# sieste/greb-climate-model

Hardware: AMD Instinct MI355X
Metric: simulated-years/sec at 96x48 grid (ensemble aggregate); diffusion HBM GB/s vs roofline (higher is better)
Workload: dtype f32; 1 GPU; 96x48 GREB ensemble, 512 members/GPU x 1 GPU, CO2 sweep 280-1120 ppm, 33 scenario years after 1 flux-correction year, dt=12h, dt_crcl=0.5h; members_per_gpu=512, arithmetic=fast, gather=none (1 GPU)

## Files before the change

### greb_climate_model_amd/csrc/greb_device.h

```cpp
#pragma once
#include <hip/hip_runtime.h>

namespace greb {

constexpr int kMaxNy = 192;

struct RowTables {
  float dif_ccy, adv_ccy;
  float dif_ccx[kMaxNy], adv_ccx[kMaxNy];
  float dif_ccx2[kMaxNy], adv_ccx2[kMaxNy];
  int dif_time2[kMaxNy], adv_time2[kMaxNy];
  int subcycled[kMaxNy];
};

struct f4 {
  float v[4];
};

typedef __attribute__((address_space(3))) float lfloat;
typedef float vfloat4 __attribute__((ext_vector_type(4)));

__device__ __forceinline__ f4 ld4(const float* p) {
  const vfloat4 a = *reinterpret_cast<const vfloat4*>(p);
  return f4{{a.x, a.y, a.z, a.w}};
}
__device__ __forceinline__ f4 ld4(const lfloat* p) {
  const vfloat4 a = *(const __attribute__((address_space(3))) vfloat4*)p;
  return f4{{a.x, a.y, a.z, a.w}};
}
__device__ __forceinline__ void st4(float* p, const f4& a) {
  vfloat4 v; v.x = a.v[0]; v.y = a.v[1]; v.z = a.v[2]; v.w = a.v[3];
  *reinterpret_cast<vfloat4*>(p) = v;
}
__device__ __forceinline__ f4 ld4_nt(const float* p) {
  const vfloat4 a = __builtin_nontemporal_load(reinterpret_cast<const vfloat4*>(p));
  return f4{{a.x, a.y, a.z, a.w}};
}
__device__ __forceinline__ void st4_nt(float* p, const f4& a) {
  vfloat4 v; v.x = a.v[0]; v.y = a.v[1]; v.z = a.v[2]; v.w = a.v[3];
  __builtin_nontemporal_store(v, reinterpret_cast<vfloat4*>(p));
}
__device__ __forceinline__ void st4(lfloat* p, const f4& a) {
  vfloat4 v; v.x = a.v[0]; v.y = a.v[1]; v.z = a.v[2]; v.w = a.v[3];
  *(__attribute__((address_space(3))) vfloat4*)p = v;
}

__device__ __forceinline__ f4 zero4() { return f4{{0.f, 0.f, 0.f, 0.f}}; }

template <typename P>
__device__ __forceinline__ void load_window(P row, int q, int nq, float t[12]) {
  const int qm = (q == 0) ? nq - 1 : q - 1;
  const int qp = (q == nq - 1) ? 0 : q + 1;
  const f4 a = ld4(row + 4 * qm), b = ld4(row + 4 * q), c = ld4(row + 4 * qp);
#pragma unroll
  for (int i = 0; i < 4; ++i) { t[i] = a.v[i]; t[4 + i] = b.v[i]; t[8 + i] = c.v[i]; }
}

__device__ __forceinline__ float min3f(float a, float b, float c) {
  float r;
  asm("v_min3_f32 %0, %1, %2, %3" : "=v"(r) : "v"(a), "v"(b), "v"(c));
  return r;
}

__device__ __forceinline__ float split_m(float u) { return u >= 0.0f ? u : 0.0f; }
__device__ __forceinline__ float split_p(float u) { return u >= 0.0f ? 0.0f : u; }


typedef float v2 __attribute__((ext_vector_type(2)));
__device__ __forceinline__ float fma_e(float a, float b, float c) { return __builtin_fmaf(a, b, c); }
__device__ __forceinline__ v2 fma_e(v2 a, v2 b, v2 c) { return __builtin_elementwise_fma(a, b, c); }
__device__ __forceinline__ float splat_e(float x, float) { return x; }
__device__ __forceinline__ v2 splat_e(float x, v2) { return v2{x, x}; }
__device__ __forceinline__ float clamp_e(float d, float T) {
#pragma clang fp contract(off)
  return (d <= -T) ? -0.9f * T : d;
}
__device__ __forceinline__ v2 clamp_e(v2 d, v2 T) { return v2{clamp_e(d.x, T.x), clamp_e(d.y, T.y)}; }

template <typename E>
__device__ __forceinline__ E div_by_const(E x, float c, float r) {
#pragma clang fp contract(off)
  const E q = x * r;
  const E e = fma_e(-q, splat_e(c, x), x);
  return fma_e(e, splat_e(r, x), q);
}
template <typename E> __device__ __forceinline__ E div20(E x) { return div_by_const(x, 20.f, 1.0f / 20.f); }
template <typename E> __device__ __forceinline__ E div3(E x) { return div_by_const(x, 3.f, 1.0f / 3.f); }

template <typename E>
__device__ __forceinline__ E dif_S_strict(const E* T, const E* w, int c) {
#pragma clang fp contract(off)
  return 10.f * (w[c - 1] * (T[c - 1] - T[c]) + w[c + 1] * (T[c + 1] - T[c]))
         + 4.f * (w[c - 2] * (T[c - 2] - T[c - 1]) + w[c - 1] * (T[c] - T[c - 1]))
         + 4.f * (w[c + 1] * (T[c] - T[c + 1]) + w[c + 2] * (T[c + 2] - T[c + 1]))
         + (w[c - 3] * (T[c - 3] - T[c - 2]) + w[c - 2] * (T[c - 1] - T[c - 2]))
         + (w[c + 2] * (T[c + 1] - T[c + 2]) + w[c + 3] * (T[c + 3] - T[c + 2]));
}

template <typename E>
__device__ __forceinline__ void dif_lon_strict(const E T[12], const E w[12], float cc, E d[4]) {
// ... 310 lines not shown
```

### greb_climate_model_amd/csrc/greb_member.hip

```cpp
#include <cstdlib>

#include "greb_kernels.h"
#include "greb_pair.h"
#include "greb_physics_step.h"
#include "greb_stencil.h"

namespace greb {

constexpr int NX = 96, NY = 48, NQ = 24, NP = 4608;
constexpr int kThreads = 512;
constexpr int RS = 2 * NX + 16;
constexpr int XB = (NY + 2) * RS;
constexpr int kOffX = RS;
constexpr int kOffW = 2 * XB + RS;
constexpr int kOffWX = 3 * XB;
constexpr int kOffWY = kOffWX + NP;
constexpr int kOffRowK = kOffWY + NP;
constexpr int kLdsFloats = kOffRowK + NY * kRowKWords;
constexpr size_t kLdsBytes = (size_t)kLdsFloats * sizeof(float);

bool member_layout_supported(const RowTables& t, int nx, int ny) {
  if (nx != NX || ny != NY) return false;
  for (int k = 0; k < NY; ++k) {
    const bool sub = (k <= 9 || k >= 38);
// ... 218 lines not shown
              "a deal must cover 3 ST, 3 FT, 1 S1 and 5 F1 passes exactly once");

__host__ __device__ constexpr int pass_tasks(int kind, int index) {
  const int total = kind == kST || kind == kFT ? 8 * NQ : (kind == kS1 ? 2 * NQ : (kind == kF1 ? 12 * NQ : 0));
  const int left = total - 64 * index;
  return left >= 64 ? 64 : (left > 0 ? left : 0);
}

template <bool STRICT>
__device__ __forceinline__ BulkTasks make_tasks(int wave, int lane) {
  BulkTasks b;
#pragma unroll
  for (int i = 0; i < 3; ++i) {
    int k = 1, q = 0, valid = 0;
    {
      const int kind = deal<STRICT>(wave, i).kind, t = deal<STRICT>(wave, i).index * 64 + lane;
      const int r = t / NQ;
      q = t % NQ;
      if (kind == kST) { valid = r < 8; k = r < 4 ? 1 + 2 * r : (r == 4 ? 41 : (r == 5 ? 39 : (r == 6 ? 45 : 43))); }
      else if (kind == kFT) { valid = r < 8; k = 10 + 2 * r; }
      else if (kind == kS1) { valid = r < 2; k = r == 0 ? 9 : 38; if (r == 1) q = (q + 4) % NQ; }
      else if (kind == kF1) { valid = r < 12; k = r < 6 ? 26 + 2 * r : 27 + 2 * (r - 6); }
      if (!valid) { k = 1; q = 0; }
    }
    TaskAddr a;
    a.c = k * RS + 4 * q;
    a.l = k * RS + 4 * (q == 0 ? NQ - 1 : q - 1);
    a.r = k * RS + 4 * (q == NQ - 1 ? 0 : q + 1);
    a.kq = valid ? (k | (q << 8)) : -1;
    asm volatile("" : "+v"(a.c), "+v"(a.l), "+v"(a.r), "+v"(a.kq));
    b.t[i] = a;
  }
  return b;
}

template <bool STRICT, int SLOT, int I>
__device__ __forceinline__ void bulk_task(lfloat* lds, int cur, const BulkTasks& tasks, int dbg, bool calm_q) {
  constexpr int kind = deal<STRICT>(SLOT, I).kind, ntask = pass_tasks(kind, deal<STRICT>(SLOT, I).index);
  if constexpr (kind != kNone && ntask > 0) {
    if (ntask < 64 && tasks.t[I].kq < 0) return;
    if constexpr (kind == kS1) { if (!(dbg & 1)) row_task<STRICT, true>(lds, cur, tasks.t[I], calm_q); }
    else if constexpr (kind == kF1) { if (!(dbg & 2)) row_task<STRICT, false>(lds, cur, tasks.t[I], calm_q); }
    else if constexpr (kind == kST) { if (!(dbg & 1)) row_task2<STRICT, true>(lds, cur, tasks.t[I], calm_q); }
    else { if (!(dbg & 2)) row_task2<STRICT, false>(lds, cur, tasks.t[I], calm_q); }
  }
}
template <bool STRICT, int SLOT>
__device__ __forceinline__ void bulk_substep(lfloat* lds, int cur, const BulkTasks& tasks, int dbg, bool calm_q = false) {
  bulk_task<STRICT, SLOT, 0>(lds, cur, tasks, dbg, calm_q);
  bulk_task<STRICT, SLOT, 1>(lds, cur, tasks, dbg, calm_q);
  bulk_task<STRICT, SLOT, 2>(lds, cur, tasks, dbg, calm_q);
}

__device__ __forceinline__ int pair_off(int l) { return (l & 1) * kHalfRow + (l >> 1) * 4; }
__device__ __forceinline__ void load_win10(const lfloat* row, int l, v2 t[10]) {
  const int lm2 = l >= 2 ? l - 2 : l + 46, lm1 = l >= 1 ? l - 1 : 47, lp1 = l <= 46 ? l + 1 : 0, lp2 = l <= 45 ? l + 2 : l - 46;
  const int idx[5] = {lm2, lm1, l, lp1, lp2};
#pragma unroll
  for (int i = 0; i < 5; ++i) {
    const vfloat4 a = *(const __attribute__((address_space(3))) vfloat4*)(row + pair_off(idx[i]));
    t[2 * i] = v2{a.x, a.y}; t[2 * i + 1] = v2{a.z, a.w};
  }
}
__device__ __forceinline__ void st_pair2(lfloat* p, v2 a, v2 b) {
  vfloat4 x; x.x = a.x; x.y = a.y; x.z = b.x; x.w = b.y;
  *(__attribute__((address_space(3))) vfloat4*)p = x;
}

__device__ __forceinline__ void chain_substep_strict(lfloat* lds, int cur, int pole, int l , bool calm_q = false) {
  if (l >= 48) return;
  const int k = pole ? NY - 1 : 0;
  const RowK rk = row_consts((const lfloat*)(lds + kOffRowK), k);
  const lfloat* Xc = lds + kOffX + cur * XB;
  const lfloat* Wc = lds + kOffW;
  v2 T0w[10], w[10];
  load_win10(Xc + k * RS, l, T0w);
  load_win10(Wc + k * RS, l, w);
  const float u0 = lds[kOffWX + k * NX + 2 * l], u1 = lds[kOffWX + k * NX + 2 * l + 1];
  const float v0 = lds[kOffWY + k * NX + 2 * l], v1 = lds[kOffWY + k * NX + 2 * l + 1];
  const int k1 = pole ? k - 1 : k + 1, k2 = pole ? k - 2 : k + 2;
  v2 T1[2], T2[2], W1[2], W2[2];
  {
    const vfloat4 a = *(const __attribute__((address_space(3))) vfloat4*)(Xc + k1 * RS + pair_off(l));
    const vfloat4 b = *(const __attribute__((address_space(3))) vfloat4*)(Xc + k2 * RS + pair_off(l));
    const vfloat4 c = *(const __attribute__((address_space(3))) vfloat4*)(Wc + k1 * RS + pair_off(l));
    const vfloat4 d = *(const __attribute__((address_space(3))) vfloat4*)(Wc + k2 * RS + pair_off(l));
    T1[0] = v2{a.x, a.y}; T1[1] = v2{a.z, a.w}; T2[0] = v2{b.x, b.y}; T2[1] = v2{b.z, b.w};
    W1[0] = v2{c.x, c.y}; W1[1] = v2{c.z, c.w}; W2[0] = v2{d.x, d.y}; W2[1] = v2{d.z, d.w};
  }
  const v2 own[2] = {T0w[4], T0w[5]};
  const bool bug_lane = (l == 46);
  const int am2 = 4 * (l >= 2 ? l - 2 : l + 46), am1 = 4 * (l >= 1 ? l - 1 : 47), ap1 = 4 * (l <= 46 ? l + 1 : 0),
            ap2 = 4 * (l <= 45 ? l + 2 : l - 46);
  auto from = [](int addr, v2 x) {
    return v2{__int_as_float(__builtin_amdgcn_ds_bpermute(addr, __float_as_int(x.x))),
              __int_as_float(__builtin_amdgcn_ds_bpermute(addr, __float_as_int(x.y)))};
  };
  const float uu[2] = {u0, u1};

  v2 Th[2][2];
#pragma unroll
  for (int which = 0; which < 2; ++which) {
    const int time2 = __builtin_amdgcn_readfirstlane(which ? rk.adv_time2 : rk.dif_time2);
    const float cc = which ? rk.adv_cc : rk.dif_cc;
    v2 T[10];
#pragma unroll
    for (int i = 0; i < 10; ++i) T[i] = T0w[i];
// ... 78 lines not shown
    constexpr int i = I, p = 3 + i;
    const int o = c.at[i >> 1] + (i & 1) * 2;
    c.w0[i] = w[p];
    c.own[i] = lds[kOffX + cur * XB + c.row[0] + o];
    c.W1[i] = Wc[c.row[1] + o];
    c.W2[i] = Wc[c.row[2] + o];
    const float u = lds[kOffWX + k * NX + 6 * j + i], v = lds[kOffWY + k * NX + 6 * j + i];
    c.cv[i] = pole == 0 ? third * fminf(v, 0.f) : -third * fmaxf(v, 0.f);
    Kd[i][0] = -csd * w[p - 3]; Kd[i][1] = (-3.f * csd) * w[p - 2]; Kd[i][2] = (-6.f * csd) * w[p - 1];
    Kd[i][3] = (6.f * csd) * w[p + 1]; Kd[i][4] = (3.f * csd) * w[p + 2]; Kd[i][5] = csd * w[p + 3];
    const float um = csa * fmaxf(u, 0.f), up = csa * fminf(u, 0.f);
    Ka[i][0] = -um * w[p - 3]; Ka[i][1] = (-4.f * um) * w[p - 2]; Ka[i][2] = (-10.f * um) * w[p - 1];
    Ka[i][3] = (-10.f * up) * w[p + 1]; Ka[i][4] = (-4.f * up) * w[p + 2]; Ka[i][5] = -up * w[p + 3];
    if (i == 3 && j == 15) {
      Ka[i][4] = -up * w[p + 3]; Ka[i][5] = -up * w[p + 3];
    }
  });
  c.kd = chain_pack(Kd);
  c.ka = chain_pack(Ka);
}

__device__ __forceinline__ void quad_chain_substep(lfloat* lds, int cur, QuadChain& c) {
  const lfloat* Xc = lds + kOffX + cur * XB;
  float own[6], T1[6], T2[6];
#pragma unroll
  for (int i = 0; i < 6; ++i) {
    const int o = c.at[i >> 1] + (i & 1) * 2;
    own[i] = c.own[i];
    T1[i] = Xc[c.row[1] + o];
    T2[i] = Xc[c.row[2] + o];
  }
  float Td[6], Ta[6];
#pragma unroll
  for (int i = 0; i < 6; ++i) { Td[i] = own[i]; Ta[i] = own[i]; }
  chain_run6<true>(Td, c.kd, c.time2_dif);
  chain_run6<true>(Ta, c.ka, c.time2_adv);
  lfloat* out = lds + kOffX + (cur ^ 1) * XB + c.row[0];
#pragma unroll
  for (int i = 0; i < 6; ++i) {
    const float g1 = c.W1[i] * (T1[i] - own[i]);
    const float d2 = c.W2[i] * (own[i] - T2[i]);
    const float ddy = c.ccy * g1;
    const float day = c.cv[i] * (d2 - g1);
    const float dd = c.w0[i] * ((Td[i] - own[i]) + ddy);
    float da = (Ta[i] - own[i]) + day;
    if (c.calm) da = 0.f;
    c.own[i] = (own[i] + dd) + da;
    out[c.at[i >> 1] + (i & 1) * 2] = c.own[i];
  }
}

template <bool STRICT>
__device__ __forceinline__ void stage_winds(lfloat* lds, const float* __restrict__ u, const float* __restrict__ v,
                                            const RowTables* __restrict__ tab) {
  constexpr int kIt = (NP / 4 + kThreads - 1) / kThreads;
  f4 uq[kIt], vq[kIt];
#pragma unroll
  for (int j = 0; j < kIt; ++j) {
    const int i = min((int)threadIdx.x + j * kThreads, NP / 4 - 1);
    uq[j] = ld4(u + 4 * i); vq[j] = ld4(v + 4 * i);
  }
#pragma unroll
  for (int j = 0; j < kIt; ++j) {
    const int i = threadIdx.x + j * kThreads;
    if (i < NP / 4) {
      const int k = i / NQ;
      if (!(STRICT || k == 0 || k == NY - 1)) {
        const RowK rk = row_consts((const lfloat*)(lds + kOffRowK), k);
        const float cu = rk.sub ? rk.adv_cc * 0.05f : rk.adv_cc * (1.f / 3.f);
        const float cv = rk.adv_ccy * (1.f / 3.f);
#pragma unroll
        for (int e = 0; e < 4; ++e) { uq[j].v[e] *= cu; vq[j].v[e] *= cv; }
      }
      st4(lds + kOffWX + 4 * i, uq[j]); st4(lds + kOffWY + 4 * i, vq[j]);
    }
  }
  (void)tab;
}

template <bool STRICT>
struct Circ {
  __device__ __forceinline__ void init(lfloat* lds, const float* wz_air, const float* wz_vapor,
                                       const RowTables* __restrict__ tab) {
    for (int i = threadIdx.x; i < 6 * RS; i += kThreads) {
      const int g = i / RS, o = i % RS;
      lds[(g >> 1) * XB + (g & 1) * (NY + 1) * RS + o] = 0.f;
    }
    stage_row_consts(lds + kOffRowK, *tab, 0, NY);
    for (int i = threadIdx.x; i < NP / 4; i += kThreads)
      st8(lds + kOffW + (i / NQ) * RS, i % NQ, zip(ld4(wz_air + 4 * i), ld4(wz_vapor + 4 * i)));
  }

  template <int WAVE>
  __device__ __forceinline__ void role_loop(lfloat* lds, int cur, int nsub, int lane, int dbg, bool calm_q
#ifdef GREB_TUNING
                                            , bool stamp, unsigned long long& busy
#endif
  ) {
    constexpr bool kPolar = is_polar_wave<STRICT>(WAVE);
    BulkTasks tasks;
    QuadChain quad;
    if constexpr (!kPolar) tasks = make_tasks<STRICT>(WAVE, lane);
    else if constexpr (!STRICT) quad_chain_setup(lds, cur, lane, calm_q, quad);
#pragma unroll 1
    for (int tt = 0; tt < nsub; ++tt) {
#ifdef GREB_TUNING
      const unsigned long long t0 = stamp ? __builtin_amdgcn_s_memtime() : 0;
#endif
      if constexpr (kPolar && STRICT) { if (!(dbg & 4)) chain_substep_strict(lds, cur, WAVE - 2, lane, calm_q); }
      else if constexpr (kPolar) { if (!(dbg & 4)) quad_chain_substep(lds, cur, quad); }
      else bulk_substep<STRICT, WAVE>(lds, cur, tasks, dbg, calm_q);
#ifdef GREB_TUNING
      if (stamp) busy += __builtin_amdgcn_s_memtime() - t0;
#endif
      __syncthreads();
      cur ^= 1;
    }
  }
  __device__ __forceinline__ void substeps(lfloat* lds, int cur, int nsub, int dbg = 0, bool calm_q = false
#ifdef GREB_TUNING
                                           , bool stamp = false, unsigned long long* busy = nullptr
#endif
  ) {
    int lane = threadIdx.x & 63;
    asm volatile("" : "+v"(lane));
#ifdef GREB_TUNING
    unsigned long long b = 0;
#define GREB_ROLE(W) case W: role_loop<W>(lds, cur, nsub, lane, dbg, calm_q, stamp, b); break;
#else
#define GREB_ROLE(W) case W: role_loop<W>(lds, cur, nsub, lane, dbg, calm_q); break;
#endif
    switch (__builtin_amdgcn_readfirstlane(threadIdx.x >> 6)) {
      GREB_ROLE(0) GREB_ROLE(1) GREB_ROLE(2) GREB_ROLE(3) GREB_ROLE(4) GREB_ROLE(5) GREB_ROLE(6) GREB_ROLE(7)
    }
#undef GREB_ROLE
#ifdef GREB_TUNING
    if (busy) *busy += b;
#endif
  }
};

template <bool STRICT>
__global__ __launch_bounds__(kThreads) void circulation_g96_kernel(const float* __restrict__ Xin,
                                                                   const float* __restrict__ wz,
                                                                   const float* __restrict__ ug,
                                                                   const float* __restrict__ vg,
                                                                   float* __restrict__ dX,
                                                                   const RowTables* __restrict__ tab, int nsub,
                                                                   int dbg) {
  extern __shared__ __align__(16) float lds_raw[];
  lfloat* lds = (lfloat*)lds_raw;
  const size_t fo = (size_t)blockIdx.x * NP;
  Circ<STRICT> c;
  c.init(lds, wz + fo, wz + fo, tab);
  for (int i = threadIdx.x; i < NP / 4; i += kThreads) {
    const f4 x = ld4(Xin + fo + 4 * i);
    st8(lds + kOffX + (i / NQ) * RS, i % NQ, zip(x, x));
  }
  __syncthreads();
  stage_winds<STRICT>(lds, ug + fo, vg + fo, tab);
  __syncthreads();
  c.substeps(lds, 0, nsub, dbg);
  const int cur = nsub & 1;
  for (int i = threadIdx.x; i < NP / 4; i += kThreads) {
    const f4 a = comp(ld8(lds + kOffX + cur * XB + (i / NQ) * RS, i % NQ), 0), b = ld4(Xin + fo + 4 * i);
    st4(dX + fo + 4 * i, f4{{a.v[0] - b.v[0], a.v[1] - b.v[1], a.v[2] - b.v[2], a.v[3] - b.v[3]}});
  }
}

hipError_t launch_circulation_g96(const float* X, const float* wz, const float* u, const float* v, float* dX,
                                  const RowTables* tab_dev, int batch, int nsub, bool strict, hipStream_t s) {
  auto kern = strict ? circulation_g96_kernel<true> : circulation_g96_kernel<false>;
  hipError_t e = hipFuncSetAttribute(reinterpret_cast<const void*>(kern),
                                     hipFuncAttributeMaxDynamicSharedMemorySize, (int)kLdsBytes);
  if (e != hipSuccess) return e;
  hipLaunchKernelGGL(kern, dim3(batch), dim3(kThreads), kLdsBytes, s, X, wz, u, v, dX, tab_dev, nsub,
                     tuning_int("GREB_DEBUG_SKIP", 0));
  return hipGetLastError();
}

template <bool STRICT, bool FLUX, bool EXP>
__global__ __launch_bounds__(kThreads) void member_kernel(MemberArgs a) {
  extern __shared__ __align__(16) float lds_raw[];
  lfloat* lds = (lfloat*)lds_raw;
  const int m = blockIdx.x, tid = threadIdx.x;
  float* state = a.state + (size_t)m * 5 * NP;
  float* acc = a.acc + (size_t)m * 6 * NP;
  float* corr = a.corr + (size_t)a.corr_index[m] * 3 * kNT * NP;
  const RowTables* tab = a.tabs + a.tab_index[m];

#ifdef GREB_TUNING
  for (int i = 0; i < (a.dbg >> 8) * (m & 7); ++i) __builtin_amdgcn_s_sleep(16);
#endif
  Circ<STRICT> circ;
  circ.init(lds, a.wz_air, a.wz_vapor, tab);
  for (int i = tid; i < NP / 4; i += kThreads)
    st8(lds + kOffX + (i / NQ) * RS, i % NQ, zip(ld4(state + NP + 4 * i), ld4(state + 3 * NP + 4 * i)));
  int cur = 0;
  __syncthreads();
#ifdef GREB_TUNING
  const bool stamp = a.stamps != nullptr;
  unsigned long long st_wind = 0, st_circ = 0, st_busy = 0, st_phys = 0;
  const unsigned long long st_c0 = stamp ? __builtin_amdgcn_s_memtime() : 0, st_r0 = stamp ? __builtin_amdgcn_s_memrealtime() : 0;
#define GREB_STAMP(var) const unsigned long long var = stamp ? __builtin_amdgcn_s_memtime() : 0
#else
#define GREB_STAMP(var)
#endif

#pragma unroll 1
  for (int s = 0; s < a.nsteps; ++s) {
    const long long it = a.it0 + s;
    const StepClock ck = step_clock<FLUX>(a, it, NP);
    const int ityr = ck.ityr, yr_rel = ck.yr_rel;
    const size_t off = ck.off;

    GREB_STAMP(t_a);
    stage_winds<STRICT>(lds, a.uclim + off, a.vclim + off, tab);
    __syncthreads();
    GREB_STAMP(t_b);

#ifdef GREB_TUNING
    circ.substeps(lds, cur, a.nsub, 0, EXP && (a.xsw & kXQDiffOnly), stamp, &st_busy);
#else
    circ.substeps(lds, cur, a.nsub, 0, EXP && (a.xsw & kXQDiffOnly));
#endif
    cur ^= a.nsub & 1;
    GREB_STAMP(t_c);

    const Phys P = a.phys[m];
    const float co2 = FLUX ? a.co2_flux : a.co2[(size_t)m * a.co2_stride + a.co2_year0 + yr_rel];
    lfloat* Xf = lds + kOffX + cur * XB;
    lfloat* red = lds + kOffX + (cur ^ 1) * XB;
#pragma unroll 1
    for (int qd = tid; qd < NP / 4; qd += kThreads) {
#ifdef GREB_TUNING
      if ((a.dbg & 4) && qd >= kThreads) break;
#endif
      const q8 xpair = ld8(Xf + (qd / NQ) * RS, qd % NQ);
      f4 oTa, oq, tsm;
      physics_quad<STRICT, FLUX, EXP>(a, P, m, qd, ck, co2, state, acc, corr, comp(xpair, 0), comp(xpair, 1), oTa, oq, tsm);
      st8(Xf + (qd / NQ) * RS, qd % NQ, zip(oTa, oq));
      if (ityr == kNT) st4(red + 4 * qd, tsm);
    }
    if (ityr == kNT) {
      __syncthreads();
      if (STRICT) {
        if (tid == 0 && a.yearly) {
#pragma clang fp contract(off)
          float sum = 0.f;
          for (int i = 0; i < NP; ++i) sum += red[i];
          float* y = a.yearly + ((size_t)m * a.yearly_years + (a.yearly_year0 + yr_rel)) * 2;
          y[0] = sum / (float)NP - 273.15f;
          y[1] = red[(a.ipy - 1) * NX + (a.ipx - 1)] - 273.15f;
        }
      } else if (a.yearly) {
        float part = 0.f;
        for (int i = tid; i < NP; i += kThreads) part += red[i];
        part = wave_sum(part);
        const float point = red[(a.ipy - 1) * NX + (a.ipx - 1)];
        __syncthreads();
        if ((tid & 63) == 0) red[tid >> 6] = part;
        __syncthreads();
        if (tid == 0) {
          float sum = 0.f;
          for (int w = 0; w < kThreads / 64; ++w) sum += red[w];
          float* y = a.yearly + ((size_t)m * a.yearly_years + (a.yearly_year0 + yr_rel)) * 2;
          y[0] = sum / (float)NP - 273.15f;
          y[1] = point - 273.15f;
        }
      }
    }
    __syncthreads();
#ifdef GREB_TUNING
    if (stamp) {
      const unsigned long long t_d = __builtin_amdgcn_s_memtime();
      st_wind += t_b - t_a; st_circ += t_c - t_b; st_phys += t_d - t_c;
    }
#endif
  }
#ifdef GREB_TUNING
  if (stamp && (tid & 63) == 0) {
    unsigned long long* o = a.stamps + ((size_t)m * (kThreads / 64) + (tid >> 6)) * 8;
    o[0] = __builtin_amdgcn_s_memtime() - st_c0; o[1] = __builtin_amdgcn_s_memrealtime() - st_r0;
    o[2] = st_wind; o[3] = st_circ; o[4] = st_busy; o[5] = st_phys; o[6] = (unsigned long long)a.nsteps; o[7] = (unsigned long long)a.nsub;
  }
#endif
}

hipError_t launch_member_kernel(const MemberArgs& a, int n_members, bool strict, hipStream_t s) {
  if (a.nx != NX || a.ny != NY) return hipErrorInvalidValue;
  void (*kern)(MemberArgs);
  if (a.xsw) {
    if (a.flux_phase) kern = strict ? member_kernel<true, true, true> : member_kernel<false, true, true>;
    else kern = strict ? member_kernel<true, false, true> : member_kernel<false, false, true>;
  } else if (a.flux_phase) kern = strict ? member_kernel<true, true, false> : member_kernel<false, true, false>;
  else kern = strict ? member_kernel<true, false, false> : member_kernel<false, false, false>;
  hipError_t e = hipFuncSetAttribute(reinterpret_cast<const void*>(kern),
                                     hipFuncAttributeMaxDynamicSharedMemorySize, (int)kLdsBytes);
  if (e != hipSuccess) return e;
  hipLaunchKernelGGL(kern, dim3(n_members), dim3(kThreads), kLdsBytes, s, a);
  return hipGetLastError();
}

}
```

### greb_climate_model_amd/csrc/greb_pair.h

```cpp
#pragma once
#include "greb_device.h"

namespace greb {


constexpr int kHalfRow = 96;
struct q8 {
  v2 v[4];
};
__device__ __forceinline__ q8 ld8(const lfloat* row, int q) {
  const vfloat4 a = *(const __attribute__((address_space(3))) vfloat4*)(row + 4 * q);
  const vfloat4 b = *(const __attribute__((address_space(3))) vfloat4*)(row + kHalfRow + 4 * q);
  q8 r;
  r.v[0] = v2{a.x, a.y}; r.v[1] = v2{a.z, a.w}; r.v[2] = v2{b.x, b.y}; r.v[3] = v2{b.z, b.w};
  return r;
}
__device__ __forceinline__ void st8(lfloat* row, int q, const q8& x) {
  vfloat4 a, b;
  a.x = x.v[0].x; a.y = x.v[0].y; a.z = x.v[1].x; a.w = x.v[1].y;
  b.x = x.v[2].x; b.y = x.v[2].y; b.z = x.v[3].x; b.w = x.v[3].y;
  *(__attribute__((address_space(3))) vfloat4*)(row + 4 * q) = a;
  *(__attribute__((address_space(3))) vfloat4*)(row + kHalfRow + 4 * q) = b;
}
__device__ __forceinline__ q8 zero8() {
  q8 r;
  r.v[0] = r.v[1] = r.v[2] = r.v[3] = v2{0.f, 0.f};
  return r;
}

__device__ __forceinline__ v2 pk_sub(v2 a, v2 b) {
  v2 r;
  asm("v_pk_add_f32 %0, %1, %2 neg_lo:[0,1] neg_hi:[0,1]" : "=v"(r) : "v"(a), "v"(b));
  return r;
}
__device__ __forceinline__ void split_sign(float u, float& pos, float& neg) {
  pos = __builtin_amdgcn_fmed3f(u, 0.f, 3.0e38f);
  neg = u - pos;
}

struct Flux2 {
  v2 Pp[10];
  v2 Pm[10];
};

__device__ __forceinline__ void make_flux2(const v2 T[12], const v2 w[12], Flux2& f) {
#pragma unroll
  for (int m = 1; m <= 9; ++m) {
    const v2 e = T[m + 1] - T[m];
    if (m >= 4) f.Pp[m] = w[m + 1] * e;
    if (m <= 6) f.Pm[m] = w[m] * e;
  }
}

__device__ __forceinline__ void dif_lon2(const Flux2& f, float cs, v2 d[4]) {
#pragma unroll
  for (int i = 0; i < 4; ++i) {
    const int c = 4 + i;
    const v2 a = f.Pp[c] - f.Pm[c - 1], b = f.Pp[c + 1] - f.Pm[c - 2], g = f.Pp[c + 2] - f.Pm[c - 3];
    d[i] = cs * (6.f * a + (3.f * b + g));
  }
}

__device__ __forceinline__ void adv_lon_full2(const Flux2& f, const v2 T[12], const v2 w[12], const float um[4],
                                              const float up[4], v2 d[4]) {
#pragma unroll
  for (int i = 0; i < 4; ++i) {
    const int c = 4 + i;
    const v2 em2 = w[c - 2] * (T[c] - T[c - 2]), ep2 = w[c + 2] * (T[c] - T[c + 2]);
    d[i] = up[i] * (ep2 - f.Pp[c]) - um[i] * (f.Pm[c - 1] + em2);
  }
}

__device__ __forceinline__ void adv_lon_sub2(const Flux2& f, const v2 T[12], const v2 w[12], const float um[4],
                                             const float up[4], bool last_quad, v2 d[4]) {
#pragma unroll
  for (int i = 0; i < 4; ++i) {
// ... 79 lines not shown
```

### greb_climate_model_amd/csrc/greb_physics_step.h

```cpp
#pragma once
#include "greb_kernels.h"

namespace greb {

__device__ __constant__ int kMonthEnd[12] = {31, 59, 90, 120, 151, 181, 212, 243, 273, 304, 334, 365};
__device__ __constant__ int kMonthDays[12] = {31, 28, 31, 30, 31, 30, 31, 31, 30, 31, 30, 31};

struct StepClock {
  int ityr, mon, yr_rel;
  size_t off, offm;
};
template <bool FLUX>
__device__ __forceinline__ StepClock step_clock(const MemberArgs& a, long long it, int np) {
  StepClock c;
  c.ityr = (int)((it - 1) % kNT) + 1;
  const int jday = (int)(((it - 1) / 2) % 365) + 1;
  c.off = (size_t)(c.ityr - 1) * np;
  c.offm = (size_t)(c.ityr > 1 ? c.ityr - 2 : kNT - 1) * np;
  c.yr_rel = (int)((it - 1) / kNT - (a.it0 - 1) / kNT);
  c.mon = -1;
  if (!FLUX && (it % 2 == 0))
    for (int mm = 0; mm < 12; ++mm) if (jday == kMonthEnd[mm]) c.mon = mm;
  return c;
}

struct PhysIn {
  f4 Ts, Ta, To, q, cap;
  f4 zt, gl, zo, ez;
  f4 tcl, cld, mld, mldm, swet, u, v;
  f4 c0, c1, c2;
  f4 acc0, acc1, acc2, acc3, acc4, acc5;
  f4 qcl, tclp;
  float solar;
};
struct PhysOut {
  f4 Ts, Ta, To, q, cap, TF, qF, ToF, tsmn;
  f4 s0, s1, s2, s3, s4;
};

template <bool FLUX, bool EXP>
__device__ __forceinline__ PhysIn physics_load(const MemberArgs& a, int qd, const StepClock& ck, const float* __restrict__ state,
                                               const float* __restrict__ acc, const float* __restrict__ corr) {
  const int nx = a.nx, ny = a.ny, np = a.np, p0 = 4 * qd;
  const size_t off = ck.off, offm = ck.offm;
  const unsigned xsw = EXP ? a.xsw : 0u;
  PhysIn i;
  i.Ts = ld4(state + p0); i.Ta = ld4(state + np + p0); i.To = ld4(state + 2 * np + p0); i.q = ld4(state + 3 * np + p0);
  i.cap = ld4(state + 4 * np + p0);
  i.zt = ld4(a.z_topo + p0); i.gl = ld4(a.glacier + p0); i.zo = ld4(a.z_ocean + p0); i.ez = ld4(a.wz_air + p0);
  i.tcl = ld4(a.tclim + off + p0); i.cld = ld4(a.cldclim + off + p0); i.mld = ld4(a.mldclim + off + p0);
  i.mldm = ld4(a.mldclim + offm + p0); i.swet = ld4(a.swetclim + off + p0); i.u = ld4(a.uclim + off + p0);
  i.v = ld4(a.vclim + off + p0);
  i.solar = a.sw_solar[(size_t)(ck.ityr - 1) * ny + p0 / nx];
  if (FLUX) { i.c0 = ld4(a.toclim + p0); i.c1 = ld4(a.qclim + off + p0); i.c2 = zero4(); }
  else { i.c0 = ld4(corr + off + p0); i.c1 = ld4(corr + (size_t)kNT * np + off + p0); i.c2 = ld4(corr + (size_t)2 * kNT * np + off + p0); }
  i.acc0 = i.acc1 = i.acc2 = i.acc3 = i.acc4 = zero4();
#ifdef GREB_TUNING
  const bool no_acc = a.dbg & 1;
#else
  constexpr bool no_acc = false;
#endif
  i.acc5 = no_acc ? zero4() : ld4(acc + 5 * np + p0);
  if (!FLUX && !no_acc) {
    i.acc0 = ld4(acc + p0); i.acc1 = ld4(acc + np + p0); i.acc2 = ld4(acc + 2 * np + p0); i.acc3 = ld4(acc + 3 * np + p0);
    i.acc4 = ld4(acc + 4 * np + p0);
  }
  i.qcl = zero4(); i.tclp = zero4();
  if (EXP && (xsw & kXLwLinear)) i.qcl = FLUX ? i.c1 : ld4(a.qclim + off + p0);
  if (EXP && !FLUX && (xsw & kXSstPlus1)) i.tclp = ld4(a.tclim + offm + p0);
  return i;
}

template <bool STRICT, bool FLUX, bool EXP>
__device__ __forceinline__ PhysOut physics_compute(const MemberArgs& a, const Phys& P, const PhysIn& in, float co2, const f4& xTa,
                                                   const f4& xq) {
  const unsigned xsw = EXP ? a.xsw : 0u;
  PhysOut o;
  o.TF = o.qF = o.ToF = zero4();
#pragma unroll
  for (int e = 0; e < 4; ++e) {
#pragma clang fp contract(off)
    float Ts1 = in.Ts.v[e];
    const float Ta1 = in.Ta.v[e], To1 = in.To.v[e], q1 = in.q.v[e], cap = in.cap.v[e];
    const float zt = in.zt.v[e], gl = in.gl.v[e], ez = in.ez.v[e], tcl = in.tcl.v[e], cld = in.cld.v[e], mld = in.mld.v[e];
    if (EXP && !FLUX && (xsw & kXSstPlus1) && zt < 0.0f) Ts1 = in.tclp.v[e] + 1.0f;
    const float dTa_crcl = xTa.v[e] - Ta1;
    const float dq_crcl = (EXP && (xsw & kXNoQTransport)) ? 0.f : xq.v[e] - q1;
    float albedo, sw, LWsurf, LWdown, em, Qlat, Qlat_air, dq_eva, dq_rain, dT_ocean, dTo;
    sw_radiation<STRICT>(P, Ts1, zt, gl, cld, in.solar, albedo, sw, xsw);
    lw_radiation<STRICT>(P, Ts1, Ta1, q1, co2, ez, cld, tcl, LWsurf, LWdown, em, xsw, in.qcl.v[e]);
    const float Qsens = P.ct_sens * (Ta1 - Ts1);
    hydro<STRICT>(P, Ts1, q1, in.u.v[e], in.v.v[e], zt, ez, in.swet.v[e], Qlat, Qlat_air, dq_eva, dq_rain, xsw);
    deep_ocean<STRICT>(P, Ts1, To1, zt, mld, in.mldm.v[e], in.zo.v[e], dT_ocean, dTo, xsw);
    const float LWup = LWdown;
    float Ts0, Ta0, To0, q0;
    if (FLUX) {
      const float dTs = fdiv<STRICT>(P.dt * (sw + LWsurf - LWdown + Qlat + Qsens), cap);
      Ts0 = Ts1 + dTs + dT_ocean;
      const float dTa = fdiv<STRICT>(P.dt * (LWup + LWdown - em * LWsurf + Qlat_air - Qsens), P.cap_air);
      Ta0 = Ta1 + dTa + dTa_crcl;
      To0 = To1 + dTo;
      const float dq = P.dt * (dq_eva + dq_rain);
      q0 = q1 + dq + dq_crcl;
      const float TF = fdiv<STRICT>((tcl - Ts0) * cap, P.dt);
      Ts0 = Ts1 + dTs + dT_ocean + fdiv<STRICT>(TF * P.dt, cap);
      const float ToF = in.c0.v[e] - To0;
      To0 = To1 + dTo + ToF;
      const float qF = in.c1.v[e] - q0;
      q0 = q1 + dq + dq_crcl + qF;
      o.TF.v[e] = TF; o.qF.v[e] = qF; o.ToF.v[e] = ToF;
    } else {
      const float TF = in.c0.v[e], qF = in.c1.v[e], ToF = in.c2.v[e];
      Ts0 = Ts1 + dT_ocean + fdiv<STRICT>(P.dt * (sw + LWsurf - LWdown + Qlat + Qsens + TF), cap);
      Ta0 = Ta1 + dTa_crcl + fdiv<STRICT>(P.dt * (LWup + LWdown - em * LWsurf + Qlat_air - Qsens), P.cap_air);
      To0 = To1 + dTo + ToF;
      float dq = P.dt * (dq_eva + dq_rain) + dq_crcl + qF;
      if (dq <= -q1) dq = -0.9f * q1;
      q0 = q1 + dq;
    }
    o.Ts.v[e] = Ts0; o.Ta.v[e] = Ta0; o.To.v[e] = To0; o.q.v[e] = q0;
    o.cap.v[e] = seaice<STRICT>(P, Ts0, zt, gl, mld, cap, xsw);
    o.tsmn.v[e] = in.acc5.v[e] + Ts0;
    o.s0.v[e] = in.acc0.v[e] + Ts0; o.s1.v[e] = in.acc1.v[e] + Ta0; o.s2.v[e] = in.acc2.v[e] + To0;
    o.s3.v[e] = in.acc3.v[e] + q0; o.s4.v[e] = in.acc4.v[e] + albedo;
  }
  return o;
}

template <bool FLUX>
__device__ __forceinline__ void physics_store(const MemberArgs& a, int m, int qd, const StepClock& ck,
                                              const PhysOut& o, float* __restrict__ state, float* __restrict__ acc,
                                              float* __restrict__ corr, f4& tsmn_mean) {
  const int np = a.np, p0 = 4 * qd, mon = ck.mon;
  const size_t off = ck.off;
#ifdef GREB_TUNING
  const bool no_acc = a.dbg & 1, no_wb = a.dbg & 2;
#else
  constexpr bool no_acc = false, no_wb = false;
#endif
  if (!no_wb) {
    st4(state + p0, o.Ts); st4(state + np + p0, o.Ta); st4(state + 2 * np + p0, o.To); st4(state + 3 * np + p0, o.q);
    st4(state + 4 * np + p0, o.cap);
  }
  if (FLUX) {
    st4(corr + off + p0, o.TF); st4(corr + (size_t)kNT * np + off + p0, o.qF); st4(corr + (size_t)2 * kNT * np + off + p0, o.ToF);
  } else {
#pragma clang fp contract(off)
    f4 s0 = o.s0, s1 = o.s1, s2 = o.s2, s3 = o.s3, s4 = o.s4;
    if (mon >= 0) {
      const float ndm = (float)(kMonthDays[mon] * 2);
      float* rec = a.monthly + (((size_t)m * a.monthly_years + (a.year_out0 + ck.yr_rel)) * 12 + mon) * 5 * np;
      f4 r0, r1, r2, r3, r4;
#pragma unroll
      for (int e = 0; e < 4; ++e) {
        r0.v[e] = s0.v[e] / ndm; r1.v[e] = s1.v[e] / ndm; r2.v[e] = s2.v[e] / ndm; r3.v[e] = s3.v[e] / ndm; r4.v[e] = s4.v[e] / ndm;
      }
      st4_nt(rec + p0, r0); st4_nt(rec + np + p0, r1); st4_nt(rec + 2 * np + p0, r2); st4_nt(rec + 3 * np + p0, r3); st4_nt(rec + 4 * np + p0, r4);
      s0 = s1 = s2 = s3 = s4 = zero4();
    }
    if (!no_acc) { st4(acc + p0, s0); st4(acc + np + p0, s1); st4(acc + 2 * np + p0, s2); st4(acc + 3 * np + p0, s3); st4(acc + 4 * np + p0, s4); }
  }
  if (ck.ityr == kNT) {
#pragma clang fp contract(off)
    f4 t;
#pragma unroll
    for (int e = 0; e < 4; ++e) t.v[e] = o.tsmn.v[e] / (float)kNT;
    tsmn_mean = t;
    if (!no_acc) st4(acc + 5 * np + p0, zero4());
  } else {
    if (!no_acc) st4(acc + 5 * np + p0, o.tsmn);
  }
}

template <bool STRICT, bool FLUX, bool EXP = false>
__device__ __forceinline__ void physics_quad(const MemberArgs& a, const Phys& P, int m, int qd, const StepClock& ck,
                                             float co2, float* __restrict__ state, float* __restrict__ acc,
                                             float* __restrict__ corr, const f4& xTa, const f4& xq, f4& oTa_out,
                                             f4& oq_out, f4& tsmn_mean) {
  const PhysIn in = physics_load<FLUX, EXP>(a, qd, ck, state, acc, corr);
  const PhysOut o = physics_compute<STRICT, FLUX, EXP>(a, P, in, co2, xTa, xq);
  physics_store<FLUX>(a, m, qd, ck, o, state, acc, corr, tsmn_mean);
  oTa_out = o.Ta; oq_out = o.q;
}

}
```

Before: 5853 simulated-years/s.

## Split physics into 3-point tasks and prefetch next-step winds after physics

The per-step physics loop now gives each thread 3 grid points instead of 4. The 1536 tasks fill three full passes of 512 threads, where the 1152 quads left the second pass partly idle. Staging of the wind fields for the next step moves to the end of the current step, sharing the existing barrier and dropping one __syncthreads per step. The trade-off is that 3-wide global loads and stores lose 16-byte vectorisation and become scalar or misaligned accesses, and LDS pair accesses are finer-grained.

Result: no change. 5841 simulated-years/s (-0.2%).

```diff
diff --git a/greb_climate_model_amd/csrc/greb_device.h b/greb_climate_model_amd/csrc/greb_device.h
--- a/greb_climate_model_amd/csrc/greb_device.h
+++ b/greb_climate_model_amd/csrc/greb_device.h
@@ -46,6 +46,37 @@
 }
 
 __device__ __forceinline__ f4 zero4() { return f4{{0.f, 0.f, 0.f, 0.f}}; }
+
+struct f3 {
+  float v[3];
+};
+template <int N> struct fvec;
+template <> struct fvec<3> { typedef f3 type; };
+template <> struct fvec<4> { typedef f4 type; };
+template <int N> using fN = typename fvec<N>::type;
+
+template <int N> __device__ __forceinline__ fN<N> ldN(const float* p) {
+  if constexpr (N == 4) return ld4(p);
+  else return f3{{p[0], p[1], p[2]}};
+}
+template <int N> __device__ __forceinline__ void stN(float* p, const fN<N>& a) {
+  if constexpr (N == 4) st4(p, a);
+  else { p[0] = a.v[0]; p[1] = a.v[1]; p[2] = a.v[2]; }
+}
+template <int N> __device__ __forceinline__ void stN_nt(float* p, const fN<N>& a) {
+  if constexpr (N == 4) st4_nt(p, a);
+  else {
+    __builtin_nontemporal_store(a.v[0], p); __builtin_nontemporal_store(a.v[1], p + 1); __builtin_nontemporal_store(a.v[2], p + 2);
+  }
+}
+template <int N> __device__ __forceinline__ void stN(lfloat* p, const fN<N>& a) {
+  if constexpr (N == 4) st4(p, a);
+  else { p[0] = a.v[0]; p[1] = a.v[1]; p[2] = a.v[2]; }
+}
+template <int N> __device__ __forceinline__ fN<N> zeroN() {
+  if constexpr (N == 4) return zero4();
+  else return f3{{0.f, 0.f, 0.f}};
+}
 
 template <typename P>
 __device__ __forceinline__ void load_window(P row, int q, int nq, float t[12]) {
diff --git a/greb_climate_model_amd/csrc/greb_member.hip b/greb_climate_model_amd/csrc/greb_member.hip
--- a/greb_climate_model_amd/csrc/greb_member.hip
+++ b/greb_climate_model_amd/csrc/greb_member.hip
@@ -294,7 +294,6 @@
   bulk_task<STRICT, SLOT, 2>(lds, cur, tasks, dbg, calm_q);
 }
 
-__device__ __forceinline__ int pair_off(int l) { return (l & 1) * kHalfRow + (l >> 1) * 4; }
 __device__ __forceinline__ void load_win10(const lfloat* row, int l, v2 t[10]) {
   const int lm2 = l >= 2 ? l - 2 : l + 46, lm1 = l >= 1 ? l - 1 : 47, lp1 = l <= 46 ? l + 1 : 0, lp2 = l <= 45 ? l + 2 : l - 46;
   const int idx[5] = {lm2, lm1, l, lp1, lp2};
@@ -479,17 +478,17 @@
 
 template <bool STRICT>
 __device__ __forceinline__ void stage_winds(lfloat* lds, const float* __restrict__ u, const float* __restrict__ v,
-                                            const RowTables* __restrict__ tab) {
+                                            const RowTables* __restrict__ tab, int tid) {
   constexpr int kIt = (NP / 4 + kThreads - 1) / kThreads;
   f4 uq[kIt], vq[kIt];
 #pragma unroll
   for (int j = 0; j < kIt; ++j) {
-    const int i = min((int)threadIdx.x + j * kThreads, NP / 4 - 1);
+    const int i = min(tid + j * kThreads, NP / 4 - 1);
     uq[j] = ld4(u + 4 * i); vq[j] = ld4(v + 4 * i);
   }
 #pragma unroll
   for (int j = 0; j < kIt; ++j) {
-    const int i = threadIdx.x + j * kThreads;
+    const int i = tid + j * kThreads;
     if (i < NP / 4) {
       const int k = i / NQ;
       if (!(STRICT || k == 0 || k == NY - 1)) {
@@ -585,7 +584,7 @@
     st8(lds + kOffX + (i / NQ) * RS, i % NQ, zip(x, x));
   }
   __syncthreads();
-  stage_winds<STRICT>(lds, ug + fo, vg + fo, tab);
+  stage_winds<STRICT>(lds, ug + fo, vg + fo, tab, threadIdx.x);
   __syncthreads();
   c.substeps(lds, 0, nsub, dbg);
   const int cur = nsub & 1;
@@ -634,16 +633,16 @@
 #define GREB_STAMP(var)
 #endif
 
+  stage_winds<STRICT>(lds, a.uclim + step_clock<FLUX>(a, a.it0, NP).off, a.vclim + step_clock<FLUX>(a, a.it0, NP).off, tab, tid);
+  __syncthreads();
+
 #pragma unroll 1
   for (int s = 0; s < a.nsteps; ++s) {
     const long long it = a.it0 + s;
     const StepClock ck = step_clock<FLUX>(a, it, NP);
     const int ityr = ck.ityr, yr_rel = ck.yr_rel;
-    const size_t off = ck.off;
-
-    GREB_STAMP(t_a);
-    stage_winds<STRICT>(lds, a.uclim + off, a.vclim + off, tab);
-    __syncthreads();
+    int tl = tid;
+    asm volatile("" : "+v"(tl));
     GREB_STAMP(t_b);
 
 #ifdef GREB_TUNING
@@ -658,16 +657,21 @@
     const float co2 = FLUX ? a.co2_flux : a.co2[(size_t)m * a.co2_stride + a.co2_year0 + yr_rel];
     lfloat* Xf = lds + kOffX + cur * XB;
     lfloat* red = lds + kOffX + (cur ^ 1) * XB;
+    constexpr int kTrRow = NX / 3;
 #pragma unroll 1
-    for (int qd = tid; qd < NP / 4; qd += kThreads) {
-#ifdef GREB_TUNING
-      if ((a.dbg & 4) && qd >= kThreads) break;
-#endif
-      const q8 xpair = ld8(Xf + (qd / NQ) * RS, qd % NQ);
-      f4 oTa, oq, tsm;
-      physics_quad<STRICT, FLUX, EXP>(a, P, m, qd, ck, co2, state, acc, corr, comp(xpair, 0), comp(xpair, 1), oTa, oq, tsm);
-      st8(Xf + (qd / NQ) * RS, qd % NQ, zip(oTa, oq));
-      if (ityr == kNT) st4(red + 4 * qd, tsm);
+    for (int t = tl; t < NP / 3; t += kThreads) {
+#ifdef GREB_TUNING
+      if ((a.dbg & 4) && t >= kThreads) break;
+#endif
+      lfloat* row = Xf + (t / kTrRow) * RS;
+      const int x0 = 3 * (t % kTrRow);
+      const int o0 = pair_at(x0), o1 = pair_at(x0 + 1), o2 = pair_at(x0 + 2);
+      const v2 x0p = ld_pair(row + o0), x1p = ld_pair(row + o1), x2p = ld_pair(row + o2);
+      f3 oTa, oq, tsm;
+      physics_quad<STRICT, FLUX, EXP, 3>(a, P, m, t, ck, co2, state, acc, corr, f3{{x0p.x, x1p.x, x2p.x}}, f3{{x0p.y, x1p.y, x2p.y}},
+                                         oTa, oq, tsm);
+      st_pair(row + o0, v2{oTa.v[0], oq.v[0]}); st_pair(row + o1, v2{oTa.v[1], oq.v[1]}); st_pair(row + o2, v2{oTa.v[2], oq.v[2]});
+      if (ityr == kNT) stN<3>(red + 3 * t, tsm);
     }
     if (ityr == kNT) {
       __syncthreads();
@@ -697,11 +701,17 @@
         }
       }
     }
+    GREB_STAMP(t_w);
+    if (s + 1 < a.nsteps) {
+      const size_t noff = step_clock<FLUX>(a, it + 1, NP).off;
+      stage_winds<STRICT>(lds, a.uclim + noff, a.vclim + noff, tab, tl);
+    }
+    GREB_STAMP(t_x);
     __syncthreads();
 #ifdef GREB_TUNING
     if (stamp) {
       const unsigned long long t_d = __builtin_amdgcn_s_memtime();
-      st_wind += t_b - t_a; st_circ += t_c - t_b; st_phys += t_d - t_c;
+      st_wind += t_x - t_w; st_circ += t_c - t_b; st_phys += (t_d - t_c) - (t_x - t_w);
     }
 #endif
   }
diff --git a/greb_climate_model_amd/csrc/greb_pair.h b/greb_climate_model_amd/csrc/greb_pair.h
--- a/greb_climate_model_amd/csrc/greb_pair.h
+++ b/greb_climate_model_amd/csrc/greb_pair.h
@@ -22,6 +22,10 @@
   *(__attribute__((address_space(3))) vfloat4*)(row + 4 * q) = a;
   *(__attribute__((address_space(3))) vfloat4*)(row + kHalfRow + 4 * q) = b;
 }
+__device__ __forceinline__ int pair_off(int l) { return (l & 1) * kHalfRow + (l >> 1) * 4; }
+__device__ __forceinline__ int pair_at(int x) { return pair_off(x >> 1) + (x & 1) * 2; }
+__device__ __forceinline__ v2 ld_pair(const lfloat* p) { return *(const __attribute__((address_space(3))) v2*)p; }
+__device__ __forceinline__ void st_pair(lfloat* p, v2 a) { *(__attribute__((address_space(3))) v2*)p = a; }
 __device__ __forceinline__ q8 zero8() {
   q8 r;
   r.v[0] = r.v[1] = r.v[2] = r.v[3] = v2{0.f, 0.f};
diff --git a/greb_climate_model_amd/csrc/greb_physics_step.h b/greb_climate_model_amd/csrc/greb_physics_step.h
--- a/greb_climate_model_amd/csrc/greb_physics_step.h
+++ b/greb_climate_model_amd/csrc/greb_physics_step.h
@@ -24,61 +24,63 @@
   return c;
 }
 
+template <int N>
 struct PhysIn {
-  f4 Ts, Ta, To, q, cap;
-  f4 zt, gl, zo, ez;
-  f4 tcl, cld, mld, mldm, swet, u, v;
-  f4 c0, c1, c2;
-  f4 acc0, acc1, acc2, acc3, acc4, acc5;
-  f4 qcl, tclp;
+  fN<N> Ts, Ta, To, q, cap;
+  fN<N> zt, gl, zo, ez;
+  fN<N> tcl, cld, mld, mldm, swet, u, v;
+  fN<N> c0, c1, c2;
+  fN<N> acc0, acc1, acc2, acc3, acc4, acc5;
+  fN<N> qcl, tclp;
   float solar;
 };
+template <int N>
 struct PhysOut {
-  f4 Ts, Ta, To, q, cap, TF, qF, ToF, tsmn;
-  f4 s0, s1, s2, s3, s4;
+  fN<N> Ts, Ta, To, q, cap, TF, qF, ToF, tsmn;
+  fN<N> s0, s1, s2, s3, s4;
 };
 
-template <bool FLUX, bool EXP>
-__device__ __forceinline__ PhysIn physics_load(const MemberArgs& a, int qd, const StepClock& ck, const float* __restrict__ state,
+template <bool FLUX, bool EXP, int N = 4>
+__device__ __forceinline__ PhysIn<N> physics_load(const MemberArgs& a, int qd, const StepClock& ck, const float* __restrict__ state,
                                                const float* __restrict__ acc, const float* __restrict__ corr) {
-  const int nx = a.nx, ny = a.ny, np = a.np, p0 = 4 * qd;
+  const int nx = a.nx, ny = a.ny, np = a.np, p0 = N * qd;
   const size_t off = ck.off, offm = ck.offm;
   const unsigned xsw = EXP ? a.xsw : 0u;
-  PhysIn i;
-  i.Ts = ld4(state + p0); i.Ta = ld4(state + np + p0); i.To = ld4(state + 2 * np + p0); i.q = ld4(state + 3 * np + p0);
-  i.cap = ld4(state + 4 * np + p0);
-  i.zt = ld4(a.z_topo + p0); i.gl = ld4(a.glacier + p0); i.zo = ld4(a.z_ocean + p0); i.ez = ld4(a.wz_air + p0);
-  i.tcl = ld4(a.tclim + off + p0); i.cld = ld4(a.cldclim + off + p0); i.mld = ld4(a.mldclim + off + p0);
-  i.mldm = ld4(a.mldclim + offm + p0); i.swet = ld4(a.swetclim + off + p0); i.u = ld4(a.uclim + off + p0);
-  i.v = ld4(a.vclim + off + p0);
+  PhysIn<N> i;
+  i.Ts = ldN<N>(state + p0); i.Ta = ldN<N>(state + np + p0); i.To = ldN<N>(state + 2 * np + p0); i.q = ldN<N>(state + 3 * np + p0);
+  i.cap = ldN<N>(state + 4 * np + p0);
+  i.zt = ldN<N>(a.z_topo + p0); i.gl = ldN<N>(a.glacier + p0); i.zo = ldN<N>(a.z_ocean + p0); i.ez = ldN<N>(a.wz_air + p0);
+  i.tcl = ldN<N>(a.tclim + off + p0); i.cld = ldN<N>(a.cldclim + off + p0); i.mld = ldN<N>(a.mldclim + off + p0);
+  i.mldm = ldN<N>(a.mldclim + offm + p0); i.swet = ldN<N>(a.swetclim + off + p0); i.u = ldN<N>(a.uclim + off + p0);
+  i.v = ldN<N>(a.vclim + off + p0);
   i.solar = a.sw_solar[(size_t)(ck.ityr - 1) * ny + p0 / nx];
-  if (FLUX) { i.c0 = ld4(a.toclim + p0); i.c1 = ld4(a.qclim + off + p0); i.c2 = zero4(); }
-  else { i.c0 = ld4(corr + off + p0); i.c1 = ld4(corr + (size_t)kNT * np + off + p0); i.c2 = ld4(corr + (size_t)2 * kNT * np + off + p0); }
-  i.acc0 = i.acc1 = i.acc2 = i.acc3 = i.acc4 = zero4();
+  if (FLUX) { i.c0 = ldN<N>(a.toclim + p0); i.c1 = ldN<N>(a.qclim + off + p0); i.c2 = zeroN<N>(); }
+  else { i.c0 = ldN<N>(corr + off + p0); i.c1 = ldN<N>(corr + (size_t)kNT * np + off + p0); i.c2 = ldN<N>(corr + (size_t)2 * kNT * np + off + p0); }
+  i.acc0 = i.acc1 = i.acc2 = i.acc3 = i.acc4 = zeroN<N>();
 #ifdef GREB_TUNING
   const bool no_acc = a.dbg & 1;
 #else
   constexpr bool no_acc = false;
 #endif
-  i.acc5 = no_acc ? zero4() : ld4(acc + 5 * np + p0);
+  i.acc5 = no_acc ? zeroN<N>() : ldN<N>(acc + 5 * np + p0);
   if (!FLUX && !no_acc) {
-    i.acc0 = ld4(acc + p0); i.acc1 = ld4(acc + np + p0); i.acc2 = ld4(acc + 2 * np + p0); i.acc3 = ld4(acc + 3 * np + p0);
-    i.acc4 = ld4(acc + 4 * np + p0);
+    i.acc0 = ldN<N>(acc + p0); i.acc1 = ldN<N>(acc + np + p0); i.acc2 = ldN<N>(acc + 2 * np + p0); i.acc3 = ldN<N>(acc + 3 * np + p0);
+    i.acc4 = ldN<N>(acc + 4 * np + p0);
   }
-  i.qcl = zero4(); i.tclp = zero4();
-  if (EXP && (xsw & kXLwLinear)) i.qcl = FLUX ? i.c1 : ld4(a.qclim + off + p0);
-  if (EXP && !FLUX && (xsw & kXSstPlus1)) i.tclp = ld4(a.tclim + offm + p0);
+  i.qcl = zeroN<N>(); i.tclp = zeroN<N>();
+  if (EXP && (xsw & kXLwLinear)) i.qcl = FLUX ? i.c1 : ldN<N>(a.qclim + off + p0);
+  if (EXP && !FLUX && (xsw & kXSstPlus1)) i.tclp = ldN<N>(a.tclim + offm + p0);
   return i;
 }
 
-template <bool STRICT, bool FLUX, bool EXP>
-__device__ __forceinline__ PhysOut physics_compute(const MemberArgs& a, const Phys& P, const PhysIn& in, float co2, const f4& xTa,
-                                                   const f4& xq) {
+template <bool STRICT, bool FLUX, bool EXP, int N>
+__device__ __forceinline__ PhysOut<N> physics_compute(const MemberArgs& a, const Phys& P, const PhysIn<N>& in, float co2, const fN<N>& xTa,
+                                                   const fN<N>& xq) {
   const unsigned xsw = EXP ? a.xsw : 0u;
-  PhysOut o;
-  o.TF = o.qF = o.ToF = zero4();
+  PhysOut<N> o;
+  o.TF = o.qF = o.ToF = zeroN<N>();
 #pragma unroll
-  for (int e = 0; e < 4; ++e) {
+  for (int e = 0; e < N; ++e) {
 #pragma clang fp contract(off)
     float Ts1 = in.Ts.v[e];
     const float Ta1 = in.Ta.v[e], To1 = in.To.v[e], q1 = in.q.v[e], cap = in.cap.v[e];
@@ -127,11 +129,11 @@
   return o;
 }
 
-template <bool FLUX>
+template <bool FLUX, int N>
 __device__ __forceinline__ void physics_store(const MemberArgs& a, int m, int qd, const StepClock& ck,
-                                              const PhysOut& o, float* __restrict__ state, float* __restrict__ acc,
-                                              float* __restrict__ corr, f4& tsmn_mean) {
-  const int np = a.np, p0 = 4 * qd, mon = ck.mon;
+                                              const PhysOut<N>& o, float* __restrict__ state, float* __restrict__ acc,
+                                              float* __restrict__ corr, fN<N>& tsmn_mean) {
+  const int np = a.np, p0 = N * qd, mon = ck.mon;
   const size_t off = ck.off;
 #ifdef GREB_TUNING
   const bool no_acc = a.dbg & 1, no_wb = a.dbg & 2;
@@ -139,46 +141,46 @@
   constexpr bool no_acc = false, no_wb = false;
 #endif
   if (!no_wb) {
-    st4(state + p0, o.Ts); st4(state + np + p0, o.Ta); st4(state + 2 * np + p0, o.To); st4(state + 3 * np + p0, o.q);
-    st4(state + 4 * np + p0, o.cap);
+    stN<N>(state + p0, o.Ts); stN<N>(state + np + p0, o.Ta); stN<N>(state + 2 * np + p0, o.To); stN<N>(state + 3 * np + p0, o.q);
+    stN<N>(state + 4 * np + p0, o.cap);
   }
   if (FLUX) {
-    st4(corr + off + p0, o.TF); st4(corr + (size_t)kNT * np + off + p0, o.qF); st4(corr + (size_t)2 * kNT * np + off + p0, o.ToF);
+    stN<N>(corr + off + p0, o.TF); stN<N>(corr + (size_t)kNT * np + off + p0, o.qF); stN<N>(corr + (size_t)2 * kNT * np + off + p0, o.ToF);
   } else {
 #pragma clang fp contract(off)
-    f4 s0 = o.s0, s1 = o.s1, s2 = o.s2, s3 = o.s3, s4 = o.s4;
+    fN<N> s0 = o.s0, s1 = o.s1, s2 = o.s2, s3 = o.s3, s4 = o.s4;
     if (mon >= 0) {
       const float ndm = (float)(kMonthDays[mon] * 2);
       float* rec = a.monthly + (((size_t)m * a.monthly_years + (a.year_out0 + ck.yr_rel)) * 12 + mon) * 5 * np;
-      f4 r0, r1, r2, r3, r4;
+      fN<N> r0, r1, r2, r3, r4;
 #pragma unroll
-      for (int e = 0; e < 4; ++e) {
+      for (int e = 0; e < N; ++e) {
         r0.v[e] = s0.v[e] / ndm; r1.v[e] = s1.v[e] / ndm; r2.v[e] = s2.v[e] / ndm; r3.v[e] = s3.v[e] / ndm; r4.v[e] = s4.v[e] / ndm;
       }
-      st4_nt(rec + p0, r0); st4_nt(rec + np + p0, r1); st4_nt(rec + 2 * np + p0, r2); st4_nt(rec + 3 * np + p0, r3); st4_nt(rec + 4 * np + p0, r4);
-      s0 = s1 = s2 = s3 = s4 = zero4();
+      stN_nt<N>(rec + p0, r0); stN_nt<N>(rec + np + p0, r1); stN_nt<N>(rec + 2 * np + p0, r2); stN_nt<N>(rec + 3 * np + p0, r3); stN_nt<N>(rec + 4 * np + p0, r4);
+      s0 = s1 = s2 = s3 = s4 = zeroN<N>();
     }
-    if (!no_acc) { st4(acc + p0, s0); st4(acc + np + p0, s1); st4(acc + 2 * np + p0, s2); st4(acc + 3 * np + p0, s3); st4(acc + 4 * np + p0, s4); }
+    if (!no_acc) { stN<N>(acc + p0, s0); stN<N>(acc + np + p0, s1); stN<N>(acc + 2 * np + p0, s2); stN<N>(acc + 3 * np + p0, s3); stN<N>(acc + 4 * np + p0, s4); }
   }
   if (ck.ityr == kNT) {
 #pragma clang fp contract(off)
-    f4 t;
+    fN<N> t;
 #pragma unroll
-    for (int e = 0; e < 4; ++e) t.v[e] = o.tsmn.v[e] / (float)kNT;
+    for (int e = 0; e < N; ++e) t.v[e] = o.tsmn.v[e] / (float)kNT;
     tsmn_mean = t;
-    if (!no_acc) st4(acc + 5 * np + p0, zero4());
+    if (!no_acc) stN<N>(acc + 5 * np + p0, zeroN<N>());
   } else {
-    if (!no_acc) st4(acc + 5 * np + p0, o.tsmn);
+    if (!no_acc) stN<N>(acc + 5 * np + p0, o.tsmn);
   }
 }
 
-template <bool STRICT, bool FLUX, bool EXP = false>
+template <bool STRICT, bool FLUX, bool EXP = false, int N = 4>
 __device__ __forceinline__ void physics_quad(const MemberArgs& a, const Phys& P, int m, int qd, const StepClock& ck,
                                              float co2, float* __restrict__ state, float* __restrict__ acc,
-                                             float* __restrict__ corr, const f4& xTa, const f4& xq, f4& oTa_out,
-                                             f4& oq_out, f4& tsmn_mean) {
-  const PhysIn in = physics_load<FLUX, EXP>(a, qd, ck, state, acc, corr);
-  const PhysOut o = physics_compute<STRICT, FLUX, EXP>(a, P, in, co2, xTa, xq);
+                                             float* __restrict__ corr, const fN<N>& xTa, const fN<N>& xq, fN<N>& oTa_out,
+                                             fN<N>& oq_out, fN<N>& tsmn_mean) {
+  const PhysIn<N> in = physics_load<FLUX, EXP, N>(a, qd, ck, state, acc, corr);
+  const PhysOut<N> o = physics_compute<STRICT, FLUX, EXP>(a, P, in, co2, xTa, xq);
   physics_store<FLUX>(a, m, qd, ck, o, state, acc, corr, tsmn_mean);
   oTa_out = o.Ta; oq_out = o.q;
 }
```
